# nanless/universal-speech-enhancement

Hardware: AMD Instinct MI355X
Metric: spectrogram-frames/sec through 30-step PC sampler, 24 kHz (higher is better)
Workload: dtype bf16; 1 GPU; configs[1]: NCSN++ Large score net, batch=8x4 s utterances per GPU, 30-step PC sampler (reverse_diffusion + langevin x1, snr 0.5, 60 NFE), bf16, hipGraph=on; global_batch=8, frames_per_utt=601, padded_frames_per_utt=640, n_freq=512, N=30, nfe=60, parallelism=utterance-sharded x1

## Files before the change

universal_speech_enhancement_amd/csrc/use_conv_v4.hip:

```cpp
#include "use_kernels.h"
#include "use_device.h"

#include <cstdio>
#include <cstdlib>

namespace use {

constexpr int V4_TW = 32, V4_TH = 16;
constexpr int V4_HW = V4_TW + 2, V4_HH = V4_TH + 2;
constexpr int V4_BN = 128;
#ifndef V4_ABL
#define V4_ABL 0
#endif
#ifndef V4_AUX_OUT
#define V4_AUX_OUT 18
#endif
#ifndef V4_AUX_IN
#define V4_AUX_IN 0
#endif
#ifndef V4_AUX_RES
#define V4_AUX_RES 2
#endif
#ifndef V4_DEAD_LOADS
#define V4_DEAD_LOADS 1
#endif

DEVI int v5_pi(int m) { return m < 4 ? m : m < 12 ? m + 4 : m - 8; }
#define V5_SW(P) ((((P) >> 2) & 1) << 1)

constexpr int v5_stg_off(int jb, int r) { return ((jb * 4 + r) * 64 + 8 * jb) * 4; }
constexpr int V5_STG_BYTES = 8448;
template <int J>
DEVI void v5_stage8(unsigned lds_base, const f32x4& x0, const f32x4& x1) {
    unsigned keep;
    asm volatile("s_mov_b32 %[keep], m0\n\ts_mov_b32 m0, %[base]\n\ts_nop 0\n\t"
                 "ds_write_addtid_b32 %[a0] offset:%[o0]\n\tds_write_addtid_b32 %[a1] offset:%[o1]\n\tds_write_addtid_b32 %[a2] offset:%[o2]\n\t"
                 "ds_write_addtid_b32 %[a3] offset:%[o3]\n\tds_write_addtid_b32 %[a4] offset:%[o4]\n\tds_write_addtid_b32 %[a5] offset:%[o5]\n\t"
                 "ds_write_addtid_b32 %[a6] offset:%[o6]\n\tds_write_addtid_b32 %[a7] offset:%[o7]\n\t"
                 "s_mov_b32 m0, %[keep]"
                 : [keep] "=&s"(keep)
                 : [base] "s"(lds_base), [a0] "v"(x0[0]), [a1] "v"(x0[1]), [a2] "v"(x0[2]), [a3] "v"(x0[3]), [a4] "v"(x1[0]), [a5] "v"(x1[1]), [a6] "v"(x1[2]), [a7] "v"(x1[3]),
                   [o0] "n"(v5_stg_off(2 * J, 0)), [o1] "n"(v5_stg_off(2 * J, 1)), [o2] "n"(v5_stg_off(2 * J, 2)), [o3] "n"(v5_stg_off(2 * J, 3)),
                   [o4] "n"(v5_stg_off(2 * J + 1, 0)), [o5] "n"(v5_stg_off(2 * J + 1, 1)), [o6] "n"(v5_stg_off(2 * J + 1, 2)), [o7] "n"(v5_stg_off(2 * J + 1, 3))
                 : "memory");
}

template <typename TIN> struct V5Xf;
#define USE_V5XF(T, MFMA, LO, HI, PK)                                                                                    \
    template <> struct V5Xf<T> {                                                                                         \
        typedef typename Mfma<T>::frag frag;                                                                             \
        DEVI static void bare8(f32x4& c0, f32x4& c1, f32x4& c2, f32x4& c3, f32x4& c4, f32x4& c5, f32x4& c6, f32x4& c7, const frag& a,       \
                               const frag& b0, const frag& b1, const frag& b2, const frag& b3, const frag& b4, const frag& b5, const frag& b6, const frag& b7) { \
            asm volatile(MFMA " %0, %8, %9, %0\n\t" MFMA " %1, %8, %10, %1\n\t" MFMA " %2, %8, %11, %2\n\t" MFMA " %3, %8, %12, %3\n\t" \
                         MFMA " %4, %8, %13, %4\n\t" MFMA " %5, %8, %14, %5\n\t" MFMA " %6, %8, %15, %6\n\t" MFMA " %7, %8, %16, %7"    \
                         : "+v"(c0), "+v"(c1), "+v"(c2), "+v"(c3), "+v"(c4), "+v"(c5), "+v"(c6), "+v"(c7)                         \
                         : "v"(a), "v"(b0), "v"(b1), "v"(b2), "v"(b3), "v"(b4), "v"(b5), "v"(b6), "v"(b7));                        \
        }                                                                                                                \
                             \
        template <bool ACT>                                                                                              \
        DEVI static void dword6(f32x4& c0, f32x4& c1, f32x4& c2, f32x4& c3, f32x4& c4, f32x4& c5, const frag& a0, const frag& a1, const frag& a2,    \
                                const frag& a3, const frag& a4, const frag& a5, const frag& b0, const frag& b1, const frag& b2, const frag& b3,     \
                                const frag& b4, const frag& b5, unsigned& d, float al, float bl, float ah, float bh) {   \
            float xl, xh, ul, uh;                                                                                        \
            if (ACT)                                                                                                     \
                asm volatile(MFMA " %0, %11, %17, %0\n\t"                                                                \
                             LO("%7", "%6") "\n\t" HI("%8", "%6") "\n\tv_fma_f32 %9, %7, %23, %24\n\t"                    \
                             MFMA " %1, %12, %18, %1\n\t"                                                                \
                             "v_fma_f32 %10, %8, %25, %26\n\tv_mul_f32 %7, 0xbfb8aa3b, %9\n\t"                            \
                             MFMA " %2, %13, %19, %2\n\t"                                                                \
                             "v_mul_f32 %8, 0xbfb8aa3b, %10\n\tv_exp_f32 %7, %7\n\tv_exp_f32 %8, %8\n\t"                  \
                             MFMA " %3, %14, %20, %3\n\t"                                                                \
                             "v_add_f32 %7, 1.0, %7\n\tv_add_f32 %8, 1.0, %8\n\t"                                        \
                             MFMA " %4, %15, %21, %4\n\t"                                                                \
                             "v_rcp_f32 %7, %7\n\tv_rcp_f32 %8, %8\n\tv_mul_f32 %9, %9, %7\n\t"                           \
                             MFMA " %5, %16, %22, %5\n\t"                                                                \
                             "v_mul_f32 %10, %10, %8\n\t" PK("%6", "%9", "%10")                                          \
                             : "+v"(c0), "+v"(c1), "+v"(c2), "+v"(c3), "+v"(c4), "+v"(c5), "+v"(d), "=&v"(xl), "=&v"(xh), "=&v"(ul), "=&v"(uh) \
                             : "v"(a0), "v"(a1), "v"(a2), "v"(a3), "v"(a4), "v"(a5), "v"(b0), "v"(b1), "v"(b2), "v"(b3), "v"(b4), "v"(b5),   \
                               "v"(al), "v"(bl), "v"(ah), "v"(bh));                                                      \
            else                                                                                                         \
                asm volatile(MFMA " %0, %11, %17, %0\n\t"                                                                \
                             LO("%7", "%6") "\n\t" HI("%8", "%6") "\n\t"                                                 \
                             MFMA " %1, %12, %18, %1\n\t"                                                                \
                             "v_fma_f32 %9, %7, %23, %24\n\tv_fma_f32 %10, %8, %25, %26\n\t"                              \
                             MFMA " %2, %13, %19, %2\n\t"                                                                \
                             MFMA " %3, %14, %20, %3\n\t"                                                                \
                             PK("%6", "%9", "%10") "\n\t"                                                                \
                             MFMA " %4, %15, %21, %4\n\t"                                                                \
                             MFMA " %5, %16, %22, %5"                                                                    \
                             : "+v"(c0), "+v"(c1), "+v"(c2), "+v"(c3), "+v"(c4), "+v"(c5), "+v"(d), "=&v"(xl), "=&v"(xh), "=&v"(ul), "=&v"(uh) \
                             : "v"(a0), "v"(a1), "v"(a2), "v"(a3), "v"(a4), "v"(a5), "v"(b0), "v"(b1), "v"(b2), "v"(b3), "v"(b4), "v"(b5),   \
                               "v"(al), "v"(bl), "v"(ah), "v"(bh));                                                      \
        }                                                                                                                \
    };
USE_V5XF(__bf16, "v_mfma_f32_16x16x32_bf16", USE_XF_BF16_LO, USE_XF_BF16_HI, USE_XF_BF16_PK)
USE_V5XF(_Float16, "v_mfma_f32_16x16x32_f16", USE_XF_F16_LO, USE_XF_F16_HI, USE_XF_F16_PK)
#undef USE_V5XF

template <typename TIN, bool ACT, typename ACC, typename AF, typename BF>
DEVI uint4 v5_mfma32_with_transform(ACC& acc, const AF& af, const BF& bf, const uint4 raw, const float (&ca)[8], const float (&cb)[8]) {
    typedef V5Xf<TIN> X;
    unsigned d[4] = {raw.x, raw.y, raw.z, raw.w};
#define V5_C(G) acc[((G) >> 4) & 1][((G) >> 3) & 1][((G) >> 1) & 3][(G)&1]
#define V5_A(G) af[((G) >> 4) & 1][((G) >> 3) & 1]
#define V5_B(G) bf[((G) >> 1) & 3][(G)&1]
    X::bare8(V5_C(0), V5_C(1), V5_C(2), V5_C(3), V5_C(4), V5_C(5), V5_C(6), V5_C(7), V5_A(0), V5_B(0), V5_B(1), V5_B(2), V5_B(3), V5_B(4), V5_B(5), V5_B(6), V5_B(7));
#define V5_D6(G0, K)                                                                                                                          \
    X::template dword6<ACT>(V5_C(G0), V5_C(G0 + 1), V5_C(G0 + 2), V5_C(G0 + 3), V5_C(G0 + 4), V5_C(G0 + 5), V5_A(G0), V5_A(G0 + 1), V5_A(G0 + 2), V5_A(G0 + 3), \
                            V5_A(G0 + 4), V5_A(G0 + 5), V5_B(G0), V5_B(G0 + 1), V5_B(G0 + 2), V5_B(G0 + 3), V5_B(G0 + 4), V5_B(G0 + 5), d[K], ca[2 * K],      \
                            cb[2 * K], ca[2 * K + 1], cb[2 * K + 1]);
    V5_D6(8, 0) V5_D6(14, 1) V5_D6(20, 2) V5_D6(26, 3)
#undef V5_D6
#undef V5_C
#undef V5_A
#undef V5_B
    return make_uint4(d[0], d[1], d[2], d[3]);
}

struct Wide32x32 {
    static constexpr int MN = 32;
    template <typename F, int K> struct Tile { typedef f32x16 acc_t[2][4]; typedef F af_t[K][2]; typedef F bf_t[K][4]; };
};
struct Wide16x16 {
    static constexpr int MN = 16;
    template <typename F, int K> struct Tile { typedef f32x4 acc_t[2][2][4][2]; typedef F af_t[2][2]; typedef F bf_t[4][2]; };
};

template <typename SHAPE, typename TIN, typename TOUT, int CK, bool ACT, int EPI>
__global__ __launch_bounds__(512) void conv_wide_kernel(ConvArgs p) {
    typedef Mfma<TIN> MF;
    constexpr bool S16 = SHAPE::MN == 16;
    static_assert(!S16 || (sizeof(TIN) == 2 && sizeof(TOUT) == 2 && CK == 32 && EPI >= 0), "Wide16x16: 16-bit storage, 32-channel chunks, specialised epilogues");
    constexpr int VEC = 16 / sizeof(TIN);
    constexpr int PARTS = CK / VEC;
    constexpr int PXB = CK * (int)sizeof(TIN);
    constexpr int BN = V4_BN, TM = 2, TN = 4;
    constexpr int KSTEPS = CK / MF::KM;
    constexpr int HROW = 48;
    constexpr int HPITCH = HROW * PXB;
    constexpr int HALO_BYTES = V4_HH * HPITCH, W_BYTES = BN * PXB;
    constexpr int MAIN_BYTES = 2 * HALO_BYTES + 2 * W_BYTES;
    constexpr int NPIECE = V4_HH * V4_HW * PARTS;
    constexpr int PIECE_ITERS = (NPIECE + 511) / 512;
    static_assert(PXB == 64, "v4 LDS layout: 64-byte rows");
    static_assert(PARTS == 4 && PIECE_ITERS == 5 && BN * PARTS == 512, "v4 staging layout");

    extern __shared__ __attribute__((aligned(16))) char smem[];
    const int tid = threadIdx.x, lane = tid & 63, wave = tid >> 6;
    const int b = blockIdx.z;
    int tile = blockIdx.x;
    if ((gridDim.x & 7) == 0) tile = (blockIdx.x & 7) * (gridDim.x >> 3) + (blockIdx.x >> 3);
    const int tiles_x = (p.W + V4_TW - 1) / V4_TW;
    const int ty0 = (tile / tiles_x) * V4_TH, tx0 = (tile % tiles_x) * V4_TW;
    const int n0 = blockIdx.y * BN;
    const int Ctot = p.C0 + p.C1, nchunks = Ctot / CK;
    const int XCtot = p.XC0 + p.XC1, nchunks2 = XCtot / CK;
    const int part = tid & (PARTS - 1);

    const int lrow = S16 ? v5_pi(lane & 15) : lane & 31;
    constexpr int NADD = TN * 32 / SHAPE::MN;
    float addv[NADD];
#pragma unroll
    for (int j = 0; j < NADD; ++j) {
        const int co = n0 + j * SHAPE::MN + lrow;
        float add = 0.f;
        if (co < p.Cout) {
            if (p.bias) add += p.bias[co];
            if (p.temb) add += p.temb[(size_t)b * p.temb_bstride + co];
        }
        addv[j] = add;
    }

#ifdef USE_HIP_TRACE_BUILD
    const bool tracing = p.trace != nullptr && (int)(blockIdx.x + gridDim.x * blockIdx.z) == p.dbg && blockIdx.y == 0 && lane == 0 && (wave & 3) == 0;
    int trace_n = 0;
    unsigned long long* const trace_lds = reinterpret_cast<unsigned long long*>(smem + 152064) + (wave >> 2) * 248;
#define V4_STAMP(ID)                                                                                   \
    if (tracing && trace_n < 124) {                                                                    \
        trace_lds[2 * trace_n] = (unsigned long long)(ID);                                             \
        trace_lds[2 * trace_n + 1] = __builtin_readcyclecounter(); ++trace_n;                          \
    }
#ifdef USE_HIP_TRACE_PHASES
#define V4_TRACE_FORCE(R) asm volatile("" :: "v"((R).x), "v"((R).y), "v"((R).z), "v"((R).w));
#define V4_PSTAMP_C(C_, ID) if ((C_) >= 1 && (C_) <= 2) { V4_STAMP(ID) }
#define V4_PSTAMP(ID) if (c >= 1 && c <= 2) { V4_STAMP(ID) }
#else
#define V4_TRACE_FORCE(R)
#define V4_PSTAMP_C(C_, ID)
#define V4_PSTAMP(ID)
#endif
#else
#define V4_STAMP(ID)
#define V4_PSTAMP(ID)
#define V4_PSTAMP_C(C_, ID)
#define V4_TRACE_FORCE(R)
#endif
    V4_STAMP(1)
    typedef typename SHAPE::template Tile<typename MF::frag, KSTEPS> RT;
    typename RT::acc_t acc;

    V4_STAMP(11)
    constexpr bool W16 = sizeof(TIN) == 2;
    const int h_ = lane >> (S16 ? 4 : 5);
#define V4_SW(P) (S16 ? V5_SW(P) : ((P) >> 2) & 3)
#define V4_KX(KK) (W16 ? ((KK) * 2) << 4 : ((KK) >> 1) << 4)
#define V4_KO(KK) (W16 ? 0 : ((KK)&1) * 8)
    int a_dx[3];
#pragma unroll
    for (int dx = 0; dx < 3; ++dx) {
        const int P = lrow + dx;
        a_dx[dx] = wave * 2 * HPITCH + P * PXB + (((W16 ? h_ : 0) ^ V4_SW(P)) << 4) + (W16 ? 0 : h_ * 4);
    }
    const int b_0 = 2 * HALO_BYTES + lrow * PXB + (((W16 ? h_ : 0) ^ ((lrow >> 2) & 3)) << 4) + (W16 ? 0 : h_ * 4);

    constexpr int COEF_OFF = MAIN_BYTES;
    constexpr int TAB_OFF = COEF_OFF + 512 * 8;
    int* const pix_tab = reinterpret_cast<int*>(smem + TAB_OFF);
    int* const dst_tab = pix_tab + PIECE_ITERS * 512;
    const int dummy_slot = ((tid / 56) * HROW + V4_HW) * PXB + (tid % 56) * 16;
    float2* const coef_lds = reinterpret_cast<float2*>(smem + COEF_OFF);
    float ca[VEC], cb[VEC];
    auto load_coef = [&](int chunk) {
        const float2* cf = coef_lds + chunk * CK + part * VEC;
#pragma unroll
        for (int k = 0; k < VEC; ++k) { const float2 v = cf[k]; ca[k] = v.x; cb[k] = v.y; }
    };
    auto buf_ld = [&](const void* base, unsigned voff, unsigned soff, int live = 1) -> uint4 {
        const __amdgpu_buffer_rsrc_t rs = __builtin_amdgcn_make_buffer_rsrc(const_cast<void*>(base), 0, live ? 0x7fffffff : 0, 0x00020000);
        return __builtin_bit_cast(uint4, __builtin_amdgcn_raw_buffer_load_b128(rs, voff, soff, 0));
    };
    auto buf_ld_in = [&](const void* base, unsigned voff, unsigned soff, int live) -> uint4 {
        const __amdgpu_buffer_rsrc_t rs = __builtin_amdgcn_make_buffer_rsrc(const_cast<void*>(base), 0, live ? 0x7fffffff : 0, 0x00020000);
        return __builtin_bit_cast(uint4, __builtin_amdgcn_raw_buffer_load_b128(rs, voff, soff, V4_AUX_IN));
    };
    auto src_ld0 = [&](int chunk, int pixoff, int live = 1) -> uint4 {
        const int c_glob = chunk * CK;
        const TIN* src; int Cs, c_loc;
        if (c_glob < p.C0) { src = (const TIN*)p.src0; Cs = p.C0; c_loc = c_glob; }
        else               { src = (const TIN*)p.src1; Cs = p.C1; c_loc = c_glob - p.C0; }
        const unsigned voff = (unsigned)pixoff * (unsigned)(Cs * (int)sizeof(TIN)) + (unsigned)(part * 16);
        return buf_ld_in(src + (size_t)b * p.H * p.W * Cs, voff, (unsigned)(c_loc * (int)sizeof(TIN)), live);
    };
    auto load_piece1 = [&](int chunk2, int q, uint4& raw) -> unsigned {
        const int pix = (q * 512 + tid) / PARTS;
        const int gy = ty0 + (pix >> 5), gx = tx0 + (pix & 31);
        const bool inb = gy < p.H && gx < p.W;
        const int c_glob = chunk2 * CK;
        const TIN* src; int Cs, c_loc;
        if (c_glob < p.XC0) { src = (const TIN*)p.x0; Cs = p.XC0; c_loc = c_glob; }
        else                { src = (const TIN*)p.x1; Cs = p.XC1; c_loc = c_glob - p.XC0; }
        const unsigned pixoff = inb ? (unsigned)(gy * p.W + gx) : 0u;
        raw = buf_ld(src + (size_t)b * p.H * p.W * Cs, pixoff * (unsigned)(Cs * (int)sizeof(TIN)) + (unsigned)(part * 16), (unsigned)(c_loc * (int)sizeof(TIN)));
        return inb ? 0xffffffffu : 0u;
    };
    auto piece1_dst = [&](int q, int hb) -> int {
        const int pix = (q * 512 + tid) / PARTS;
        const int P = ((pix >> 5) + 1) * HROW + (pix & 31) + 1;
        return hb * HALO_BYTES + P * PXB + ((part ^ V4_SW(P)) << 4);
    };

    const unsigned wvoff = (unsigned)tid * 16u;
    const int wdst = 2 * HALO_BYTES + tid * 16;
    const unsigned slab_b = (unsigned)(p.cout_pad * CK) * (unsigned)sizeof(TIN);
    const unsigned n0_b = (unsigned)(n0 * CK) * (unsigned)sizeof(TIN);
#define V4_LOAD_W(CC, TT, R)                                                                                         \
    {                                                                                                                \
        const int cw0_ = (TT) > 8 ? (CC) + 1 : (CC);                                                                 \
        const int cw_ = cw0_ < nchunks ? cw0_ : nchunks - 1;  \
        const int tw_ = (TT) > 8 ? (TT)-9 : (TT);             \
        R = buf_ld(p.wb, wvoff, (unsigned)(tw_ * nchunks + cw_) * slab_b + n0_b, V4_DEAD_LOADS ? (cw0_ < nchunks) : 1);       \
    }
#define V4_STORE_W(BUF, R) { *reinterpret_cast<uint4*>(smem + (BUF)*W_BYTES + wdst) = R; }

    uint4 wS, hL[3];
    const uint4 zero4 = make_uint4(0, 0, 0, 0);
    wS = hL[0] = hL[1] = hL[2] = zero4;
    {
        V4_STAMP(12)
        uint4 w0 = zero4, raw[PIECE_ITERS];
        float2 cfv = make_float2(1.f, 0.f);
        if (tid < Ctot)
            cfv = p.gn_st0 ? gn_coef_of(p.gn_st0, p.C0, p.gn_st1, p.C1, p.gn_gamma, p.gn_beta, p.gn_groups, p.gn_inv_n, p.gn_eps, b, tid)
                  : p.coef ? *reinterpret_cast<const float2*>(p.coef + ((size_t)b * Ctot + tid) * 2) : make_float2(1.f, 0.f);
        V4_LOAD_W(0, 0, w0);
        V4_LOAD_W(0, 1, wS);
        int slot[PIECE_ITERS], ppv[PIECE_ITERS]; bool inbv[PIECE_ITERS];
#pragma unroll
        for (int j = 0; j < PIECE_ITERS; ++j) {
            const int idx = j * 512 + tid;
            const int pix = idx < NPIECE ? idx / PARTS : 0;
            const int hy = pix / V4_HW, hx = pix - hy * V4_HW;
            const int gy = ty0 + hy - 1, gx = tx0 + hx - 1;
            const bool inb = idx < NPIECE && gy >= 0 && gy < p.H && gx >= 0 && gx < p.W;
            int pp = inb ? gy * p.W + gx : 0;
#ifdef USE_HIP_ABLATE_HALO
            pp = idx & 127;
#endif
#ifdef USE_HIP_ABLATE
            if (p.dbg & 1) pp = idx & 127;
#endif
            raw[j] = (V4_ABL & 32) ? zero4 : src_ld0(0, pp);
            const int P = hy * HROW + hx;
            slot[j] = P * PXB + ((part ^ V4_SW(P)) << 4);
            ppv[j] = pp; inbv[j] = inb;
            if (idx >= NPIECE) slot[j] = -1;
        }
        __builtin_amdgcn_sched_barrier(0);
        V4_STAMP(13)
#pragma unroll
        for (int j = 0; j < PIECE_ITERS; ++j) {
            const int idx = j * 512 + tid;
            if (slot[j] >= 0 && !inbv[j]) {
                *reinterpret_cast<uint4*>(smem + slot[j]) = zero4;
                *reinterpret_cast<uint4*>(smem + HALO_BYTES + slot[j]) = zero4;
            }
            pix_tab[idx] = ppv[j];
            slot[j] = inbv[j] ? slot[j] : dummy_slot;
            dst_tab[idx] = slot[j];
        }
#pragma unroll
        for (int i = 0; i < TM; ++i)
#pragma unroll
            for (int j = 0; j < TN; ++j)
#pragma unroll
                for (int r = 0; r < 16; ++r) {
                    if constexpr (S16) acc[i][(r >> 3) & 1][j][(r >> 2) & 1][r & 3] = addv[2 * j + ((r >> 2) & 1)];
                    else acc[i][j][r] = addv[j];
                }
        if (tid < Ctot) coef_lds[tid] = cfv;
        V4_STAMP(14)
        __syncthreads();
        V4_STAMP(15)
        load_coef(0);
        V4_STORE_W(0, w0);
        V4_STAMP(16)
#pragma unroll
        for (int j = 0; j < PIECE_ITERS; ++j)
            *reinterpret_cast<uint4*>(smem + slot[j]) = (V4_ABL & 32) ? raw[j] : stage_transform<TIN, ACT>(raw[j], 0xffffffffu, ca, cb);
    }

    typename RT::af_t af; typename RT::bf_t bf;
    int dst_ = 0;
    uint4 tkeep = zero4; int dkeep = 0;
#ifdef USE_HIP_SETPRIO
#define V4_SETPRIO(N) __builtin_amdgcn_s_setprio(N);
#else
#define V4_SETPRIO(N)
#endif
#ifdef V4_PEEL_LAST
#define V4_P0 1
#else
#define V4_P0 0
#define V4_STG 1
#endif
#define V4_LD_PHASE(T) (V4_STG && (T) >= V4_P0 && (T) < PIECE_ITERS + V4_P0)
#define V4_XF_PHASE(T) (V4_STG && (T) >= V4_P0 + 2 && (T) < PIECE_ITERS + V4_P0 + 2)
#define V4_XF_IDX(T) (V4_XF_PHASE(T) ? (T) - V4_P0 - 2 : 0)
#define V4_LD_FRAGS(HA_, WB_, DX, GUARD)                                                                             \
    if constexpr (S16) {                                                                                             \
        _Pragma("unroll") for (int i = 0; i < TM; ++i)                                                               \
            _Pragma("unroll") for (int a = 0; a < 2; ++a) af[i][a] = MF::ld((HA_) + a_dx[DX] + i * HPITCH + a * 16 * PXB); \
        _Pragma("unroll") for (int j = 0; j < TN; ++j)                                                               \
            _Pragma("unroll") for (int bb = 0; bb < 2; ++bb) bf[j][bb] = MF::ld((WB_) + b_0 + (2 * j + bb) * 16 * PXB); \
    } else {                                                                                                         \
        _Pragma("unroll") for (int kk = 0; kk < KSTEPS; ++kk) {                                                      \
            int ak_ = a_dx[DX], bk_ = b_0;                                                                           \
            if ((GUARD) && !W16) asm volatile("" : "+v"(ak_), "+v"(bk_));    \
            ak_ ^= V4_KX(kk); bk_ ^= V4_KX(kk);                                                                      \
            _Pragma("unroll") for (int i = 0; i < TM; ++i) af[kk][i] = MF::ld((HA_) + ak_ + i * HPITCH + V4_KO(kk)); \
            _Pragma("unroll") for (int j = 0; j < TN; ++j) bf[kk][j] = MF::ld((WB_) + bk_ + j * 32 * PXB + V4_KO(kk)); \
        }                                                                                                            \
    }
#define V4_LDS(CC, T)                                                                                                \
    {                                                                                                                \
        const int cc_ = (CC);                                                                                        \
        const int par_ = cc_ & 1;                             \
        const int cn_ = cc_ + 1 < nchunks ? cc_ + 1 : cc_;    \
        int pix_ = 0;                                         \
                                                        \
        if (V4_LD_PHASE(T)) pix_ = (V4_ABL & 128) ? tid * 3 : pix_tab[(V4_LD_PHASE(T) ? (T) - V4_P0 : 0) * 512 + tid]; \
        if (V4_XF_PHASE(T)) dst_ = (V4_ABL & 128) ? tid * 80 : dst_tab[V4_XF_IDX(T) * 512 + tid];    \
        {                                                                                                            \
            const char* ha_ = smem + par_ * HALO_BYTES + ((T) / 3) * HPITCH;                                         \
            const char* wbuf_ = smem + (par_ ^ ((T)&1)) * W_BYTES;                                                   \
            if (!(V4_ABL & 8) || ((CC) == 0 && (T) == 0)) { V4_LD_FRAGS(ha_, wbuf_, (T) % 3, true) }                 \
        }                                                                                                            \
        __builtin_amdgcn_sched_barrier(0);                                                                           \
        if (!S16 && (V4_ABL & 512) && (T) >= 3 + V4_P0 && (T) < PIECE_ITERS + 3 + V4_P0) *reinterpret_cast<uint4*>(smem + dkeep) = tkeep;    \
        if (V4_XF_PHASE(T)) dst_ += (par_ ^ 1) * HALO_BYTES;           \
        if ((V4_ABL & 256) && V4_XF_PHASE(T)) dst_ = (par_ ^ 1) * HALO_BYTES + tid * 16;                             \
        if (!(V4_ABL & 4)) {                                                                                         \
        V4_STORE_W((par_ ^ ((T)&1)) ^ 1, wS);                                                                        \
        V4_LOAD_W(cc_, (T) + 2, wS);                                                                                 \
        }                                                                                                            \
        __builtin_amdgcn_sched_barrier(0);                         \
        if (V4_LD_PHASE(T)) {                                                                                        \
            if ((T) == V4_P0) load_coef(cn_);                                                                        \
            hL[((T) - V4_P0) % 3] = src_ld0(cn_, pix_, V4_DEAD_LOADS ? (cc_ + 1 < nchunks) : 1);                                                         \
        }                                                                                                            \
    }
#define V4_MMA_ALL()                                                                                                 \
    if constexpr (S16) {                                                                                             \
        _Pragma("unroll") for (int i = 0; i < TM; ++i)                                                               \
            _Pragma("unroll") for (int a = 0; a < 2; ++a)                                                            \
                V5Xf<TIN>::bare8(acc[i][a][0][0], acc[i][a][0][1], acc[i][a][1][0], acc[i][a][1][1], acc[i][a][2][0], acc[i][a][2][1], acc[i][a][3][0], acc[i][a][3][1], \
                                 af[i][a], bf[0][0], bf[0][1], bf[1][0], bf[1][1], bf[2][0], bf[2][1], bf[3][0], bf[3][1]); \
    } else {                                                                                                         \
        _Pragma("unroll") for (int kk = 0; kk < KSTEPS; ++kk)                                                        \
            _Pragma("unroll") for (int i = 0; i < TM; ++i)                                                           \
                _Pragma("unroll") for (int j = 0; j < TN; ++j) acc[i][j] = MF::mma(af[kk][i], bf[kk][j], acc[i][j]); \
    }
#define V4_MFMA(CC, T)                                                                                               \
    {                                                                                                                \
        V4_SETPRIO(1)                                                                                                \
        if constexpr (sizeof(TIN) == 2) {                 \
            if (V4_XF_PHASE(T)) {                      \
                                 \
                V4_PSTAMP_C(CC, 300 + (T))       \
                V4_TRACE_FORCE(hL[V4_XF_IDX(T) % 3])                                                                 \
                V4_PSTAMP_C(CC, 400 + (T))                                                                           \
                if (V4_ABL & 1) {                                                                                    \
                    V4_MMA_ALL()                                                                                     \
                    if (!(V4_ABL & 64)) *reinterpret_cast<uint4*>(smem + dst_) = hL[V4_XF_IDX(T) % 3];               \
                } else {                                                                                             \
                    uint4 t0;                                                                                        \
                    if constexpr (S16) t0 = v5_mfma32_with_transform<TIN, ACT>(acc, af, bf, hL[V4_XF_IDX(T) % 3], ca, cb); \
                    else t0 = mfma16_with_transform<TIN, ACT>(acc, af, bf, hL[V4_XF_IDX(T) % 3], ca, cb);            \
                    if (!S16 && (V4_ABL & 512)) { tkeep = t0; asm volatile("" : "+v"(tkeep.x), "+v"(tkeep.y), "+v"(tkeep.z), "+v"(tkeep.w)); dkeep = dst_; } \
                    else if (!(V4_ABL & 64)) *reinterpret_cast<uint4*>(smem + dst_) = t0;  \
                }                                                                                                    \
            } else {                                                                                                 \
                V4_MMA_ALL()                                                                                         \
            }                                                                                                        \
        } else {                                                                                                     \
            V4_MMA_ALL()                                                                                             \
            if (V4_XF_PHASE(T)) {                                                                                    \
                const uint4 t0 = stage_transform<TIN, ACT>(hL[V4_XF_IDX(T) % 3], 0xffffffffu, ca, cb);               \
                *reinterpret_cast<uint4*>(smem + dst_) = t0;                                                         \
                _Pragma("unroll") for (int g = 0; g < 16; ++g) {                                                     \
                    __builtin_amdgcn_sched_group_barrier(0x008, TM * TN * KSTEPS / 16, 0);                \
                    __builtin_amdgcn_sched_group_barrier(0x002, 3, 0);                                  \
                    __builtin_amdgcn_sched_group_barrier(0x400, 1, 0);                                  \
                }                                                                                                    \
            }                                                                                                        \
        }                                                                                                            \
        V4_SETPRIO(0)                                                                                                \
    }

#define V4_BAR() { __builtin_amdgcn_sched_barrier(0); __syncthreads(); __builtin_amdgcn_sched_barrier(0); }
#define V4_BAR_M() { __builtin_amdgcn_sched_barrier(0); asm volatile("s_barrier" ::: "memory"); __builtin_amdgcn_sched_barrier(0); }
    V4_STAMP(2)
    V4_BAR();
    V4_STAMP(3)
#define V4_G0_CHUNK(LAST)                                                                                            \
            V4_STAMP(50 + c)                                                                                         \
            V4_G0_STEP(0) V4_G0_STEP(1) V4_G0_STEP(2) V4_G0_STEP(3) V4_G0_STEP(4) V4_G0_STEP(5) V4_G0_STEP(6) V4_G0_STEP(7) \
            V4_MFMA(c, 8)                                                                                            \
            V4_BAR_M();                                                                                              \
            if (!(LAST) && c + 1 < nchunks) V4_LDS(c + 1, 0)     \
            V4_BAR();
#define V4_G0_STEP(T) V4_MFMA(c, T) V4_PSTAMP(100 + (T)) V4_BAR_M(); V4_LDS(c, (T) + 1) V4_PSTAMP(200 + (T) + 1) V4_BAR();
#define V4_G1_STEP(T) V4_LDS(c, T) V4_PSTAMP(200 + (T)) V4_BAR(); V4_MFMA(c, T) V4_PSTAMP(100 + (T)) V4_BAR_M();
#define V4_G1_CHUNK                                                                                                  \
            V4_STAMP(50 + c)                                                                                         \
            V4_G1_STEP(0) V4_G1_STEP(1) V4_G1_STEP(2) V4_G1_STEP(3) V4_G1_STEP(4) V4_G1_STEP(5) V4_G1_STEP(6) V4_G1_STEP(7) V4_G1_STEP(8)
#ifdef V4_PEEL_LAST
#define V4_STG 1
    if (wave < 4) {
        V4_LDS(0, 0)
        V4_BAR();
        for (int c = 0; c < nchunks - 1; ++c) { V4_G0_CHUNK(false) }
#undef V4_STG
#define V4_STG 0
        { const int c = nchunks - 1; V4_G0_CHUNK(true) }
    } else {
        V4_BAR();
#undef V4_STG
#define V4_STG 1
        for (int c = 0; c < nchunks - 1; ++c) { V4_G1_CHUNK }
#undef V4_STG
#define V4_STG 0
        { const int c = nchunks - 1; V4_G1_CHUNK }
    }
#undef V4_STG
#define V4_STG 1
#else
    if (wave < 4) {
        V4_LDS(0, 0)
        V4_BAR();
        for (int c = 0; c < nchunks; ++c) { V4_G0_CHUNK(false) }
    } else {
        V4_BAR();
        for (int c = 0; c < nchunks; ++c) { V4_G1_CHUNK }
    }
#endif
#undef V4_G0_STEP
#undef V4_G1_STEP
#undef V4_G0_CHUNK
#undef V4_G1_CHUNK
#undef V4_BAR
#undef V4_BAR_M
#undef V4_LDS
#undef V4_LOAD_W

    V4_STAMP(4)
    if (V4_ABL & 16) {
        float sum = 0.f;
#pragma unroll
        for (int i = 0; i < TM; ++i)
#pragma unroll
            for (int j = 0; j < TN; ++j)
#pragma unroll
                for (int r = 0; r < 16; ++r) {
                    if constexpr (S16) sum += acc[i][(r >> 3) & 1][j][(r >> 2) & 1][r & 3];
                    else sum += acc[i][j][r];
                }
        if (sum == 1.2345f) ((float*)p.out)[tid] = sum;
        return;
    }
    if (nchunks2 > 0) {
        uint4 r0, r1, r2, r3, wa; unsigned m0, m1, m2, m3;
        const unsigned slab2_b = (unsigned)(p.cout_pad * CK) * (unsigned)sizeof(TIN);
#define V4_SC_LOAD(C2)                                                                                        \
        {                                                                                                     \
            m0 = load_piece1(C2, 0, r0); m1 = load_piece1(C2, 1, r1); m2 = load_piece1(C2, 2, r2); m3 = load_piece1(C2, 3, r3); \
            wa = buf_ld(p.w2b, wvoff, (unsigned)(C2)*slab2_b + n0_b);                                         \
        }
        V4_SC_LOAD(0)
        for (int c2 = 0; c2 < nchunks2; ++c2) {
            const int buf = c2 & 1;
            r0.x &= m0; r0.y &= m0; r0.z &= m0; r0.w &= m0; r1.x &= m1; r1.y &= m1; r1.z &= m1; r1.w &= m1;
            r2.x &= m2; r2.y &= m2; r2.z &= m2; r2.w &= m2; r3.x &= m3; r3.y &= m3; r3.z &= m3; r3.w &= m3;
            *reinterpret_cast<uint4*>(smem + piece1_dst(0, buf)) = r0; *reinterpret_cast<uint4*>(smem + piece1_dst(1, buf)) = r1;
            *reinterpret_cast<uint4*>(smem + piece1_dst(2, buf)) = r2; *reinterpret_cast<uint4*>(smem + piece1_dst(3, buf)) = r3;
            V4_STORE_W(buf, wa);
            __syncthreads();
            if (c2 + 1 < nchunks2) V4_SC_LOAD(c2 + 1)
            const char* ha_ = smem + buf * HALO_BYTES + HPITCH;
            const char* wb2_ = smem + buf * W_BYTES;
            V4_LD_FRAGS(ha_, wb2_, 1, false)
            V4_MFMA(nchunks, 0)
        }
#undef V4_SC_LOAD
    }
    V4_STAMP(5)
    __syncthreads();
    V4_STAMP(6)
#undef V4_MFMA
#undef V4_MMA_ALL
#undef V4_XF_PHASE
#undef V4_STORE_W
#undef V4_LD_FRAGS
#undef V4_KX
#undef V4_KO
#undef V4_SW

    constexpr int STG_LD = BN + 4;
    constexpr bool ATID = S16 || (EPI >= 0 && !(EPI & 4) && sizeof(TOUT) == 2);
    constexpr int STG_WAVE = S16 ? V5_STG_BYTES : ATID ? V4_STG_ATID_BYTES : 32 * STG_LD * 4;
    static_assert(!ATID || 7 * STG_WAVE < 65536, "conv_wide: wave-7 staging base exceeds M0[15:0]");
    constexpr int CH = 16 / (int)sizeof(TOUT);
    constexpr int CPR = BN / CH;
    constexpr int QN = 32 * CPR / 64;
    constexpr int PPP = 64 / CPR;
    float* const stg = reinterpret_cast<float*>(smem + wave * STG_WAVE);
    float* const red = reinterpret_cast<float*>(smem + 8 * STG_WAVE);
    const int ch = lane % CPR;
    const int co0 = n0 + ch * CH;
    const bool cok = co0 < p.Cout;
    const int wave_u = __builtin_amdgcn_readfirstlane(wave);
    const size_t img_elems = (size_t)p.H * p.W * p.Cout;
    const __amdgpu_buffer_rsrc_t rs_out = __builtin_amdgcn_make_buffer_rsrc((TOUT*)p.out + (size_t)b * img_elems, 0, 0x7fffffff, 0x00020000);
    const __amdgpu_buffer_rsrc_t rs_res = __builtin_amdgcn_make_buffer_rsrc(const_cast<TOUT*>((const TOUT*)p.res) + (size_t)b * img_elems, 0, 0x7fffffff, 0x00020000);
    const unsigned voff = cok ? (unsigned)(((lane / CPR) * p.Cout + co0) * (int)sizeof(TOUT)) : 0x80000000u;
    const unsigned pass_b = (unsigned)(PPP * p.Cout) * (unsigned)sizeof(TOUT);
    constexpr bool EPI_RT = EPI < 0;
    const bool has_res = EPI_RT ? p.res != nullptr : (EPI & 1) != 0;
    const bool has_scale = EPI_RT ? p.out_scale != 1.f : (EPI & 2) != 0;
    const bool has_pyr = EPI_RT ? p.pyr != nullptr : (EPI & 4) != 0;
    constexpr bool HOIST_W4 = sizeof(TOUT) == 2;
    float4 w4r[CH]; float b4r[CH];
    if (HOIST_W4 && has_pyr && cok) {
#pragma unroll
        for (int c = 0; c < CH; ++c) { w4r[c] = *reinterpret_cast<const float4*>(p.w4 + (size_t)(co0 + c) * 4); b4r[c] = p.b4[co0 + c]; }
    } else {
#pragma unroll
        for (int c = 0; c < CH; ++c) { w4r[c] = make_float4(0.f, 0.f, 0.f, 0.f); b4r[c] = 0.f; }
    }
    f32x2 st_s2[CH / 2], st_q2[CH / 2];
#pragma unroll
    for (int k = 0; k < CH / 2; ++k) { st_s2[k] = (f32x2){0.f, 0.f}; st_q2[k] = (f32x2){0.f, 0.f}; }
    const float* const stg_rd = S16    ? stg + ((ch >> 1) * 4 + (lane >> 4)) * 64 + 8 * (ch >> 1) + ((ch & 1) ? 4 : 0)
                                : ATID ? stg + (ch >> 2) * 512 + (lane >> 4) * 64 + 4 * (((ch >> 2) & 1) + 8 * (ch >> 3)) + (ch & 3) * 8
                                       : stg + (lane / CPR) * STG_LD + ch * CH;
    const float* const stg_rd1 = stg + ((ch >> 1) * 4 + (lane >> 4)) * 64 + 8 * (ch >> 1) + ((ch & 1) ? 8 : 12);
    auto stg_rd_ptr = [&](int q, int c4) -> const float* {
        const int ql = q & 3;
        return S16    ? (c4 ? stg_rd1 : stg_rd) + 16 * (ql == 0 ? 0 : ql == 1 ? 3 : ql == 2 ? 1 : 2)
               : ATID ? stg_rd + ((q >> 1) & 1) * 256 + (q & 1) * 32 + c4 * 4
                      : stg_rd + q * PPP * STG_LD + c4 * 4;
    };
    const unsigned stg_lds = (unsigned)(size_t)(__attribute__((address_space(3))) char*)smem + (unsigned)(wave_u * STG_WAVE);
    auto row_bytes = [&](int i) -> unsigned {
        return (unsigned)(((ty0 + wave_u * 2 + i) * p.W + tx0) * p.Cout) * (unsigned)sizeof(TOUT);
    };
    auto res_load = [&](int i, uint4 (&rv)[QN]) {
        const unsigned row_b = row_bytes(i);
#pragma unroll
        for (int q = 0; q < QN; ++q)
            rv[q] = (V4_ABL & 8192) ? make_uint4(q, q, q, q) : __builtin_bit_cast(uint4, __builtin_amdgcn_raw_buffer_load_b128(rs_res, voff + row_b + (unsigned)q * pass_b, 0, V4_AUX_RES));
    };
    auto stage_write = [&](int i) {
        if constexpr (!S16) {
#pragma unroll
            for (int j = 0; j < TN; ++j)
#pragma unroll
                for (int r = 0; r < 16; ++r) {
                    const int row = (r & 3) + 8 * (r >> 2) + 4 * (lane >> 5);
                    stg[row * STG_LD + j * 32 + (lane & 31)] = acc[i][j][r];
                }
        }
    };
    constexpr int NQ = S16 ? QN / 2 : EPI_RT ? 1 : (EPI & 4) ? QN / 4 : ATID ? QN / 2 : QN;
    auto stage_write_half = [&](int i, int hb) {
        if constexpr (S16) {
            v5_stage8<0>(stg_lds, acc[i][hb][0][0], acc[i][hb][0][1]); v5_stage8<1>(stg_lds, acc[i][hb][1][0], acc[i][hb][1][1]);
            v5_stage8<2>(stg_lds, acc[i][hb][2][0], acc[i][hb][2][1]); v5_stage8<3>(stg_lds, acc[i][hb][3][0], acc[i][hb][3][1]);
        } else if (hb == 0) { v4_stage8<0, 0>(stg_lds, acc[i][0]); v4_stage8<1, 0>(stg_lds, acc[i][1]); v4_stage8<2, 0>(stg_lds, acc[i][2]); v4_stage8<3, 0>(stg_lds, acc[i][3]); }
        else                { v4_stage8<0, 8>(stg_lds, acc[i][0]); v4_stage8<1, 8>(stg_lds, acc[i][1]); v4_stage8<2, 8>(stg_lds, acc[i][2]); v4_stage8<3, 8>(stg_lds, acc[i][3]); }
    };
    auto stage_read = [&](int q0, f32x4 (&t)[NQ][CH / 4]) {
#pragma unroll
        for (int q = 0; q < NQ; ++q)
#pragma unroll
            for (int c4 = 0; c4 < CH / 4; ++c4) t[q][c4] = *reinterpret_cast<const f32x4*>(stg_rd_ptr(q0 + q, c4));
    };
    auto finish = [&](int i, int q0, const f32x4 (&t)[NQ][CH / 4], const uint4 (&rv)[QN]) {
        const int gy = ty0 + wave_u * 2 + i;
        const unsigned row_b = row_bytes(i);
        float4 pq[NQ];
        if (has_pyr) {
#pragma unroll
            for (int q = 0; q < NQ; ++q) {
                const size_t pix = (size_t)(b * p.H + gy) * p.W + tx0 + ((q0 + q) * 64 + lane) / CPR;
                pq[q] = *reinterpret_cast<const float4*>(p.pyr + pix * 4);
            }
        }
#pragma unroll
        for (int q = 0; q < NQ; ++q) {
            f32x2 v2[CH / 2];
#pragma unroll
            for (int c4 = 0; c4 < CH / 4; ++c4) { v2[c4 * 2] = (f32x2){t[q][c4].x, t[q][c4].y}; v2[c4 * 2 + 1] = (f32x2){t[q][c4].z, t[q][c4].w}; }
            if (has_res) {
                float rvf[CH];
                Vec16<TOUT>::load(reinterpret_cast<const TOUT*>(&rv[q0 + q]), rvf);
#pragma unroll
                for (int k = 0; k < CH / 2; ++k) v2[k] += (f32x2){rvf[2 * k], rvf[2 * k + 1]};
            }
            if (has_scale) {
#pragma unroll
                for (int k = 0; k < CH / 2; ++k) v2[k] *= (f32x2){p.out_scale, p.out_scale};
            }
            float v[CH];
#pragma unroll
            for (int k = 0; k < CH / 2; ++k) { v[2 * k] = v2[k].x; v[2 * k + 1] = v2[k].y; }
            if (has_pyr) {
#pragma unroll
                for (int c = 0; c < CH; ++c) {
                    const float4 wq = HOIST_W4 ? w4r[c] : (cok ? *reinterpret_cast<const float4*>(p.w4 + (size_t)(co0 + c) * 4) : make_float4(0.f, 0.f, 0.f, 0.f));
                    v[c] += (HOIST_W4 ? b4r[c] : (cok ? p.b4[co0 + c] : 0.f)) + wq.x * pq[q].x + wq.y * pq[q].y + wq.z * pq[q].z + wq.w * pq[q].w;
                }
            }
            if (!EPI_RT || cok) {
            const uint4 packed = Vec16<TOUT>::pack(v);
            if (V4_ABL & 1024) asm volatile("" :: "v"(packed.x), "v"(packed.y), "v"(packed.z), "v"(packed.w));
            else
            __builtin_amdgcn_raw_buffer_store_b128(__builtin_bit_cast(__attribute__((ext_vector_type(4))) unsigned, packed), rs_out,
                                                   voff + row_b + (unsigned)(q0 + q) * pass_b, 0, V4_AUX_OUT);
            if (!(V4_ABL & 4096)) {
#pragma unroll
                for (int k = 0; k < CH / 2; ++k) {
                    const f32x2 x = {v[2 * k], v[2 * k + 1]};
                    st_s2[k] += x; st_q2[k] = __builtin_elementwise_fma(x, x, st_q2[k]);
                }
            }
            }
        }
    };
    {
        uint4 rv0[QN], rv1[QN];
        f32x4 t[NQ][CH / 4];
        if (has_res) res_load(0, rv0);
        if constexpr (ATID) {
            static_assert(NQ * (CH / 4) == 8 && QN == 8, "8 pieces per half round");
            auto pin = [&]() {
                asm volatile("" : "+v"(t[0][0]), "+v"(t[0][1]), "+v"(t[1][0]), "+v"(t[1][1]), "+v"(t[2][0]), "+v"(t[2][1]), "+v"(t[3][0]), "+v"(t[3][1]) :: "memory");
                __builtin_amdgcn_sched_barrier(0);
            };
            auto fence = [&]() { asm volatile("" ::: "memory"); __builtin_amdgcn_sched_barrier(0); };
            constexpr bool RV2 = !(EPI & 4);
            stage_write_half(0, 0);
            stage_read(0, t); if (has_res && RV2) res_load(1, rv1); pin();
            stage_write_half(0, 1); fence();
// ... 170 lines not shown
```

Before: 3682 spectrogram-frames/s.

## Spread S16 conv input transform across multiple MFMA phases with new load/store schedule

For the S16 wide-conv path, the per-dword normalize/SiLU transform that was packed into one phase is now distributed across phases 2–7, interleaved with MFMA chains of configurable length (6/7/8/10 per dword). The halo loads and the transformed stores get their own phase tables, so stores happen in phases 3–7 instead of right after the transform. The aim is to hide the transcendental and VALU work under more MFMA issue slots and reduce the stall in a single dense phase. In exchange, register lifetimes of hL grow, the schedule becomes more complex, and there is a risk of register pressure or mistimed LDS writes.

```diff
diff --git a/universal_speech_enhancement_amd/csrc/use_conv_v4.hip b/universal_speech_enhancement_amd/csrc/use_conv_v4.hip
--- a/universal_speech_enhancement_amd/csrc/use_conv_v4.hip
+++ b/universal_speech_enhancement_amd/csrc/use_conv_v4.hip
@@ -45,6 +45,53 @@
                  : "memory");
 }
 
+#define V5_MF(MFMA, N) MFMA " %[c" #N "], %[a" #N "], %[b" #N "], %[c" #N "]\n\t"
+#define V5_I0(LO) LO("%[xl]", "%[d]") "\n\t"
+#define V5_I1(HI) HI("%[xh]", "%[d]") "\n\t"
+#define V5_I2 "v_fma_f32 %[ul], %[xl], %[al], %[bl]\n\t"
+#define V5_I3 "v_fma_f32 %[uh], %[xh], %[ah], %[bh]\n\t"
+#define V5_I4 "v_mul_f32 %[xl], 0xbfb8aa3b, %[ul]\n\t"
+#define V5_I5 "v_mul_f32 %[xh], 0xbfb8aa3b, %[uh]\n\t"
+#define V5_I6 "v_exp_f32 %[xl], %[xl]\n\t"
+#define V5_I7 "v_exp_f32 %[xh], %[xh]\n\t"
+#define V5_I8 "v_add_f32 %[xl], 1.0, %[xl]\n\t"
+#define V5_I9 "v_add_f32 %[xh], 1.0, %[xh]\n\t"
+#define V5_I10 "v_rcp_f32 %[xl], %[xl]\n\t"
+#define V5_I11 "v_rcp_f32 %[xh], %[xh]\n\t"
+#define V5_I12 "v_mul_f32 %[ul], %[ul], %[xl]\n\t"
+#define V5_I13 "v_mul_f32 %[uh], %[uh], %[xh]\n\t"
+#define V5_I14(PK) PK("%[d]", "%[ul]", "%[uh]")
+#define V5_ACT1(S) S
+#define V5_ACT0(S)
+#define V5_BODY10(W, MFMA, LO, HI, PK)                                                                                   \
+    V5_MF(MFMA, 0) V5_I0(LO) V5_I1(HI) V5_MF(MFMA, 1) V5_I2 V5_I3 V5_MF(MFMA, 2) W(V5_I4 V5_I5) V5_MF(MFMA, 3) W(V5_I6) V5_MF(MFMA, 4) W(V5_I7)  \
+    V5_MF(MFMA, 5) W(V5_I8 V5_I9) V5_MF(MFMA, 6) W(V5_I10) V5_MF(MFMA, 7) W(V5_I11) V5_MF(MFMA, 8) W(V5_I12 V5_I13) V5_MF(MFMA, 9) V5_I14(PK)
+#define V5_BODY8(W, MFMA, LO, HI, PK)                                                                                    \
+    V5_MF(MFMA, 0) V5_I0(LO) V5_I1(HI) V5_MF(MFMA, 1) V5_I2 V5_I3 V5_MF(MFMA, 2) W(V5_I4 V5_I5) V5_MF(MFMA, 3) W(V5_I6) V5_MF(MFMA, 4) W(V5_I7 V5_I8) \
+    V5_MF(MFMA, 5) W(V5_I9 V5_I10) V5_MF(MFMA, 6) W(V5_I11 V5_I12) V5_MF(MFMA, 7) W(V5_I13) V5_I14(PK)
+#define V5_BODY7(W, MFMA, LO, HI, PK)                                                                                    \
+    V5_MF(MFMA, 0) V5_I0(LO) V5_I1(HI) V5_MF(MFMA, 1) V5_I2 V5_I3 V5_MF(MFMA, 2) W(V5_I4 V5_I5 V5_I6) V5_MF(MFMA, 3) W(V5_I7 V5_I8)              \
+    V5_MF(MFMA, 4) W(V5_I9 V5_I10) V5_MF(MFMA, 5) W(V5_I11 V5_I12) V5_MF(MFMA, 6) W(V5_I13) V5_I14(PK)
+#define V5_BODY6(W, MFMA, LO, HI, PK)                                                                                    \
+    V5_MF(MFMA, 0) V5_I0(LO) V5_I1(HI) V5_I2 V5_MF(MFMA, 1) V5_I3 W(V5_I4) V5_MF(MFMA, 2) W(V5_I5 V5_I6 V5_I7) V5_MF(MFMA, 3) W(V5_I8 V5_I9)     \
+    V5_MF(MFMA, 4) W(V5_I10 V5_I11 V5_I12) V5_MF(MFMA, 5) W(V5_I13) V5_I14(PK)
+#define V5_C(G) acc[((G) >> 4) & 1][((G) >> 3) & 1][((G) >> 1) & 3][(G)&1]
+#define V5_A(G) af[((G) >> 4) & 1][((G) >> 3) & 1]
+#define V5_B(G) bf[((G) >> 1) & 3][(G)&1]
+#define V5_O(N) [c##N] "+v"(V5_C(G0 + N))
+#define V5_N(N) [a##N] "v"(V5_A(G0 + N)), [b##N] "v"(V5_B(G0 + N))
+#define V5_OUT6 V5_O(0), V5_O(1), V5_O(2), V5_O(3), V5_O(4), V5_O(5)
+#define V5_OUT7 V5_OUT6, V5_O(6)
+#define V5_OUT8 V5_OUT7, V5_O(7)
+#define V5_OUT10 V5_OUT8, V5_O(8), V5_O(9)
+#define V5_IN6 V5_N(0), V5_N(1), V5_N(2), V5_N(3), V5_N(4), V5_N(5)
+#define V5_IN7 V5_IN6, V5_N(6)
+#define V5_IN8 V5_IN7, V5_N(7)
+#define V5_IN10 V5_IN8, V5_N(8), V5_N(9)
+#define V5_UNIT(K, W, MFMA, LO, HI, PK)                                                                                  \
+    asm volatile(V5_BODY##K(W, MFMA, LO, HI, PK)                                                                         \
+                 : V5_OUT##K, [d] "+v"(d), [xl] "=&v"(xl), [xh] "=&v"(xh), [ul] "=&v"(ul), [uh] "=&v"(uh)                  \
+                 : V5_IN##K, [al] "v"(al), [bl] "v"(bl), [ah] "v"(ah), [bh] "v"(bh))
 template <typename TIN> struct V5Xf;
 #define USE_V5XF(T, MFMA, LO, HI, PK)                                                                                    \
     template <> struct V5Xf<T> {                                                                                         \
@@ -56,65 +103,48 @@
                          : "+v"(c0), "+v"(c1), "+v"(c2), "+v"(c3), "+v"(c4), "+v"(c5), "+v"(c6), "+v"(c7)                         \
                          : "v"(a), "v"(b0), "v"(b1), "v"(b2), "v"(b3), "v"(b4), "v"(b5), "v"(b6), "v"(b7));                        \
         }                                                                                                                \
-                             \
-        template <bool ACT>                                                                                              \
-        DEVI static void dword6(f32x4& c0, f32x4& c1, f32x4& c2, f32x4& c3, f32x4& c4, f32x4& c5, const frag& a0, const frag& a1, const frag& a2,    \
-                                const frag& a3, const frag& a4, const frag& a5, const frag& b0, const frag& b1, const frag& b2, const frag& b3,     \
-                                const frag& b4, const frag& b5, unsigned& d, float al, float bl, float ah, float bh) {   \
+        DEVI static void mfma(f32x4& c, const frag& a, const frag& b) { asm volatile(MFMA " %0, %1, %2, %0" : "+v"(c) : "v"(a), "v"(b)); }     \
+                                             \
+        template <bool ACT, int K, int G0, typename ACC, typename AF, typename BF>                                       \
+        DEVI static void unit(ACC& acc, const AF& af, const BF& bf, unsigned& d, float al, float bl, float ah, float bh) {                    \
+            static_assert(K == 6 || K == 7 || K == 8 || K == 10, "cuts of the chain: 6, 7, 8 or 10 MFMAs per dword");     \
             float xl, xh, ul, uh;                                                                                        \
-            if (ACT)                                                                                                     \
-                asm volatile(MFMA " %0, %11, %17, %0\n\t"                                                                \
-                             LO("%7", "%6") "\n\t" HI("%8", "%6") "\n\tv_fma_f32 %9, %7, %23, %24\n\t"                    \
-                             MFMA " %1, %12, %18, %1\n\t"                                                                \
-                             "v_fma_f32 %10, %8, %25, %26\n\tv_mul_f32 %7, 0xbfb8aa3b, %9\n\t"                            \
-                             MFMA " %2, %13, %19, %2\n\t"                                                                \
-                             "v_mul_f32 %8, 0xbfb8aa3b, %10\n\tv_exp_f32 %7, %7\n\tv_exp_f32 %8, %8\n\t"                  \
-                             MFMA " %3, %14, %20, %3\n\t"                                                                \
-                             "v_add_f32 %7, 1.0, %7\n\tv_add_f32 %8, 1.0, %8\n\t"                                        \
-                             MFMA " %4, %15, %21, %4\n\t"                                                                \
-                             "v_rcp_f32 %7, %7\n\tv_rcp_f32 %8, %8\n\tv_mul_f32 %9, %9, %7\n\t"                           \
-                             MFMA " %5, %16, %22, %5\n\t"                                                                \
-                             "v_mul_f32 %10, %10, %8\n\t" PK("%6", "%9", "%10")                                          \
-                             : "+v"(c0), "+v"(c1), "+v"(c2), "+v"(c3), "+v"(c4), "+v"(c5), "+v"(d), "=&v"(xl), "=&v"(xh), "=&v"(ul), "=&v"(uh) \
-                             : "v"(a0), "v"(a1), "v"(a2), "v"(a3), "v"(a4), "v"(a5), "v"(b0), "v"(b1), "v"(b2), "v"(b3), "v"(b4), "v"(b5),   \
-                               "v"(al), "v"(bl), "v"(ah), "v"(bh));                                                      \
-            else                                                                                                         \
-                asm volatile(MFMA " %0, %11, %17, %0\n\t"                                                                \
-                             LO("%7", "%6") "\n\t" HI("%8", "%6") "\n\t"                                                 \
-                             MFMA " %1, %12, %18, %1\n\t"                                                                \
-                             "v_fma_f32 %9, %7, %23, %24\n\tv_fma_f32 %10, %8, %25, %26\n\t"                              \
-                             MFMA " %2, %13, %19, %2\n\t"                                                                \
-                             MFMA " %3, %14, %20, %3\n\t"                                                                \
-                             PK("%6", "%9", "%10") "\n\t"                                                                \
-                             MFMA " %4, %15, %21, %4\n\t"                                                                \
-                             MFMA " %5, %16, %22, %5"                                                                    \
-                             : "+v"(c0), "+v"(c1), "+v"(c2), "+v"(c3), "+v"(c4), "+v"(c5), "+v"(d), "=&v"(xl), "=&v"(xh), "=&v"(ul), "=&v"(uh) \
-                             : "v"(a0), "v"(a1), "v"(a2), "v"(a3), "v"(a4), "v"(a5), "v"(b0), "v"(b1), "v"(b2), "v"(b3), "v"(b4), "v"(b5),   \
-                               "v"(al), "v"(bl), "v"(ah), "v"(bh));                                                      \
+            if constexpr (K == 10) { if constexpr (ACT) V5_UNIT(10, V5_ACT1, MFMA, LO, HI, PK); else V5_UNIT(10, V5_ACT0, MFMA, LO, HI, PK); } \
+            else if constexpr (K == 8) { if constexpr (ACT) V5_UNIT(8, V5_ACT1, MFMA, LO, HI, PK); else V5_UNIT(8, V5_ACT0, MFMA, LO, HI, PK); } \
+            else if constexpr (K == 7) { if constexpr (ACT) V5_UNIT(7, V5_ACT1, MFMA, LO, HI, PK); else V5_UNIT(7, V5_ACT0, MFMA, LO, HI, PK); } \
+            else { if constexpr (ACT) V5_UNIT(6, V5_ACT1, MFMA, LO, HI, PK); else V5_UNIT(6, V5_ACT0, MFMA, LO, HI, PK); }   \
         }                                                                                                                \
     };
 USE_V5XF(__bf16, "v_mfma_f32_16x16x32_bf16", USE_XF_BF16_LO, USE_XF_BF16_HI, USE_XF_BF16_PK)
 USE_V5XF(_Float16, "v_mfma_f32_16x16x32_f16", USE_XF_F16_LO, USE_XF_F16_HI, USE_XF_F16_PK)
 #undef USE_V5XF
 
-template <typename TIN, bool ACT, typename ACC, typename AF, typename BF>
-DEVI uint4 v5_mfma32_with_transform(ACC& acc, const AF& af, const BF& bf, const uint4 raw, const float (&ca)[8], const float (&cb)[8]) {
-    typedef V5Xf<TIN> X;
-    unsigned d[4] = {raw.x, raw.y, raw.z, raw.w};
-#define V5_C(G) acc[((G) >> 4) & 1][((G) >> 3) & 1][((G) >> 1) & 3][(G)&1]
-#define V5_A(G) af[((G) >> 4) & 1][((G) >> 3) & 1]
-#define V5_B(G) bf[((G) >> 1) & 3][(G)&1]
-    X::bare8(V5_C(0), V5_C(1), V5_C(2), V5_C(3), V5_C(4), V5_C(5), V5_C(6), V5_C(7), V5_A(0), V5_B(0), V5_B(1), V5_B(2), V5_B(3), V5_B(4), V5_B(5), V5_B(6), V5_B(7));
-#define V5_D6(G0, K)                                                                                                                          \
-    X::template dword6<ACT>(V5_C(G0), V5_C(G0 + 1), V5_C(G0 + 2), V5_C(G0 + 3), V5_C(G0 + 4), V5_C(G0 + 5), V5_A(G0), V5_A(G0 + 1), V5_A(G0 + 2), V5_A(G0 + 3), \
-                            V5_A(G0 + 4), V5_A(G0 + 5), V5_B(G0), V5_B(G0 + 1), V5_B(G0 + 2), V5_B(G0 + 3), V5_B(G0 + 4), V5_B(G0 + 5), d[K], ca[2 * K],      \
-                            cb[2 * K], ca[2 * K + 1], cb[2 * K + 1]);
-    V5_D6(8, 0) V5_D6(14, 1) V5_D6(20, 2) V5_D6(26, 3)
-#undef V5_D6
-#undef V5_C
-#undef V5_A
-#undef V5_B
-    return make_uint4(d[0], d[1], d[2], d[3]);
+#ifndef V5_SCHED
+#define V5_SCHED 0
+#endif
+constexpr int v5_xf_d0(int t) { return t < 2 || t > 7 ? 0 : t < 6 ? 3 * (t - 2) : 12 + 4 * (t - 6); }
+constexpr int v5_xf_nd(int t) { return t < 2 || t > 7 ? 0 : t < 6 ? 3 : 4; }
+constexpr int v5_xf_head(int t) { return V5_SCHED == 1 || (t == 2 && V5_SCHED < 2) ? 8 : t < 6 ? 2 : V5_SCHED == 3 ? 0 : 4; }
+constexpr int v5_xf_k(int t) { return V5_SCHED == 1 ? (t < 6 ? 8 : 6) : t == 2 && V5_SCHED < 2 ? 8 : t < 6 ? 10 : V5_SCHED == 3 ? 8 : 7; }
+constexpr int v5_ld_piece(int t) { return t >= 0 && t <= 2 ? t : t == 4 || t == 5 ? t - 1 : -1; }
+constexpr int v5_st_piece(int t) { return t >= 3 && t <= 7 ? t - 3 : -1; }
+
+template <int C> DEVI unsigned& v5_comp(uint4& v) {
+    if constexpr (C == 0) return v.x; else if constexpr (C == 1) return v.y; else if constexpr (C == 2) return v.z; else return v.w;
+}
+template <typename TIN, bool ACT, int HEAD, int K, int D0, int ND, int G = 0, typename ACC, typename AF, typename BF>
+DEVI void v5_mfma32_spread(ACC& acc, const AF& af, const BF& bf, uint4 (&hL)[3], const float (&ca)[8], const float (&cb)[8]) {
+    static_assert(HEAD + K * ND <= 32, "a phase has 32 MFMAs");
+    if constexpr (G < 32) {
+        if constexpr (G >= HEAD && G < HEAD + K * ND) {
+            constexpr int n = D0 + (G - HEAD) / K, q = n & 3;
+            V5Xf<TIN>::template unit<ACT, K, G>(acc, af, bf, v5_comp<q>(hL[(n >> 2) % 3]), ca[2 * q], cb[2 * q], ca[2 * q + 1], cb[2 * q + 1]);
+            v5_mfma32_spread<TIN, ACT, HEAD, K, D0, ND, G + K>(acc, af, bf, hL, ca, cb);
+        } else {
+            V5Xf<TIN>::mfma(V5_C(G), V5_A(G), V5_B(G));
+            v5_mfma32_spread<TIN, ACT, HEAD, K, D0, ND, G + 1>(acc, af, bf, hL, ca, cb);
+        }
+    }
 }
 
 struct Wide32x32 {
@@ -353,9 +383,13 @@
 #define V4_P0 0
 #define V4_STG 1
 #endif
-#define V4_LD_PHASE(T) (V4_STG && (T) >= V4_P0 && (T) < PIECE_ITERS + V4_P0)
+#define V4_LD32_PHASE(T) (V4_STG && (T) >= V4_P0 && (T) < PIECE_ITERS + V4_P0)
 #define V4_XF_PHASE(T) (V4_STG && (T) >= V4_P0 + 2 && (T) < PIECE_ITERS + V4_P0 + 2)
 #define V4_XF_IDX(T) (V4_XF_PHASE(T) ? (T) - V4_P0 - 2 : 0)
+#define V4_LD_PHASE(T) (S16 ? V4_STG && v5_ld_piece(T) >= 0 : V4_LD32_PHASE(T))
+#define V4_LD_IDX(T) (S16 ? (v5_ld_piece(T) >= 0 ? v5_ld_piece(T) : 0) : V4_LD32_PHASE(T) ? (T) - V4_P0 : 0)
+#define V4_ST_PHASE(T) (S16 ? V4_STG && v5_st_piece(T) >= 0 : V4_XF_PHASE(T))
+#define V4_ST_IDX(T) (S16 ? (v5_st_piece(T) >= 0 ? v5_st_piece(T) : 0) : V4_XF_IDX(T))
 #define V4_LD_FRAGS(HA_, WB_, DX, GUARD)                                                                             \
     if constexpr (S16) {                                                                                             \
         _Pragma("unroll") for (int i = 0; i < TM; ++i)                                                               \
@@ -378,8 +412,8 @@
         const int cn_ = cc_ + 1 < nchunks ? cc_ + 1 : cc_;    \
         int pix_ = 0;                                         \
                                                         \
-        if (V4_LD_PHASE(T)) pix_ = (V4_ABL & 128) ? tid * 3 : pix_tab[(V4_LD_PHASE(T) ? (T) - V4_P0 : 0) * 512 + tid]; \
-        if (V4_XF_PHASE(T)) dst_ = (V4_ABL & 128) ? tid * 80 : dst_tab[V4_XF_IDX(T) * 512 + tid];    \
+        if (V4_LD_PHASE(T)) pix_ = (V4_ABL & 128) ? tid * 3 : pix_tab[V4_LD_IDX(T) * 512 + tid];                    \
+        if (V4_ST_PHASE(T)) dst_ = (V4_ABL & 128) ? tid * 80 : dst_tab[V4_ST_IDX(T) * 512 + tid];    \
         {                                                                                                            \
             const char* ha_ = smem + par_ * HALO_BYTES + ((T) / 3) * HPITCH;                                         \
             const char* wbuf_ = smem + (par_ ^ ((T)&1)) * W_BYTES;                                                   \
@@ -387,16 +421,16 @@
         }                                                                                                            \
         __builtin_amdgcn_sched_barrier(0);                                                                           \
         if (!S16 && (V4_ABL & 512) && (T) >= 3 + V4_P0 && (T) < PIECE_ITERS + 3 + V4_P0) *reinterpret_cast<uint4*>(smem + dkeep) = tkeep;    \
-        if (V4_XF_PHASE(T)) dst_ += (par_ ^ 1) * HALO_BYTES;           \
-        if ((V4_ABL & 256) && V4_XF_PHASE(T)) dst_ = (par_ ^ 1) * HALO_BYTES + tid * 16;                             \
+        if (V4_ST_PHASE(T)) dst_ += (par_ ^ 1) * HALO_BYTES;           \
+        if ((V4_ABL & 256) && V4_ST_PHASE(T)) dst_ = (par_ ^ 1) * HALO_BYTES + tid * 16;                             \
         if (!(V4_ABL & 4)) {                                                                                         \
         V4_STORE_W((par_ ^ ((T)&1)) ^ 1, wS);                                                                        \
         V4_LOAD_W(cc_, (T) + 2, wS);                                                                                 \
         }                                                                                                            \
         __builtin_amdgcn_sched_barrier(0);                         \
         if (V4_LD_PHASE(T)) {                                                                                        \
-            if ((T) == V4_P0) load_coef(cn_);                                                                        \
-            hL[((T) - V4_P0) % 3] = src_ld0(cn_, pix_, V4_DEAD_LOADS ? (cc_ + 1 < nchunks) : 1);                                                         \
+            if (V4_LD_IDX(T) == 0) load_coef(cn_);                                                                   \
+            hL[V4_LD_IDX(T) % 3] = src_ld0(cn_, pix_, V4_DEAD_LOADS ? (cc_ + 1 < nchunks) : 1);                                                         \
         }                                                                                                            \
     }
 #define V4_MMA_ALL()                                                                                                 \
@@ -413,7 +447,21 @@
 #define V4_MFMA(CC, T)                                                                                               \
     {                                                                                                                \
         V4_SETPRIO(1)                                                                                                \
-        if constexpr (sizeof(TIN) == 2) {                 \
+        if constexpr (S16) {                                                                                         \
+            if constexpr (V4_STG && v5_xf_nd(T) > 0) {  \
+                V4_PSTAMP_C(CC, 300 + (T))  \
+                V4_TRACE_FORCE(hL[(v5_xf_d0(T) >> 2) % 3])                                                           \
+                V4_PSTAMP_C(CC, 400 + (T))                                                                           \
+                if (V4_ABL & 1) {                                                                                    \
+                    V4_MMA_ALL()                                                                                     \
+                } else {                                                                                             \
+                    v5_mfma32_spread<TIN, ACT, v5_xf_head(T), v5_xf_k(T), v5_xf_d0(T), v5_xf_nd(T)>(acc, af, bf, hL, ca, cb); \
+                }                                                                                                    \
+                if (V4_ST_PHASE(T) && !(V4_ABL & 64)) *reinterpret_cast<uint4*>(smem + dst_) = hL[V4_ST_IDX(T) % 3];  \
+            } else {                                                                                                 \
+                V4_MMA_ALL()                                                                                         \
+            }                                                                                                        \
+        } else if constexpr (sizeof(TIN) == 2) {          \
             if (V4_XF_PHASE(T)) {                      \
                                  \
                 V4_PSTAMP_C(CC, 300 + (T))       \
@@ -424,8 +472,7 @@
                     if (!(V4_ABL & 64)) *reinterpret_cast<uint4*>(smem + dst_) = hL[V4_XF_IDX(T) % 3];               \
                 } else {                                                                                             \
                     uint4 t0;                                                                                        \
-                    if constexpr (S16) t0 = v5_mfma32_with_transform<TIN, ACT>(acc, af, bf, hL[V4_XF_IDX(T) % 3], ca, cb); \
-                    else t0 = mfma16_with_transform<TIN, ACT>(acc, af, bf, hL[V4_XF_IDX(T) % 3], ca, cb);            \
+                    t0 = mfma16_with_transform<TIN, ACT>(acc, af, bf, hL[V4_XF_IDX(T) % 3], ca, cb);            \
                     if (!S16 && (V4_ABL & 512)) { tkeep = t0; asm volatile("" : "+v"(tkeep.x), "+v"(tkeep.y), "+v"(tkeep.z), "+v"(tkeep.w)); dkeep = dst_; } \
                     else if (!(V4_ABL & 64)) *reinterpret_cast<uint4*>(smem + dst_) = t0;  \
                 }                                                                                                    \
@@ -549,6 +596,8 @@
 #undef V4_MFMA
 #undef V4_MMA_ALL
 #undef V4_XF_PHASE
+#undef V4_LD_PHASE
+#undef V4_ST_PHASE
 #undef V4_STORE_W
 #undef V4_LD_FRAGS
 #undef V4_KX
```

Result: no change. 3704 spectrogram-frames/s (median of 6 runs) (+0.6%).
